# mit-han-lab/distrifuser

Measured on NVIDIA H100. Metric: SDXL 50-step latency (ms/image), lower is better.
Workload: dtype f16

## Files before the change

### distrifuser_b200/compat/unet_2d_condition.py

```python
from __future__ import annotations

import math
from types import SimpleNamespace

import torch
from torch import nn
from torch.nn import functional as F

SDXL = dict(
    in_channels=4, out_channels=4, block_out_channels=(320, 640, 1280), layers_per_block=2,
    down_block_types=("DownBlock2D", "CrossAttnDownBlock2D", "CrossAttnDownBlock2D"),
    up_block_types=("CrossAttnUpBlock2D", "CrossAttnUpBlock2D", "UpBlock2D"),
    transformer_layers_per_block=(1, 2, 10), attention_head_dim=(5, 10, 20), cross_attention_dim=2048,
    use_linear_projection=True, norm_num_groups=32, norm_eps=1e-5, addition_embed_type="text_time",
    addition_time_embed_dim=256, projection_class_embeddings_input_dim=2816, sample_size=128,
)
SD15 = dict(
    in_channels=4, out_channels=4, block_out_channels=(320, 640, 1280, 1280), layers_per_block=2,
    down_block_types=("CrossAttnDownBlock2D",) * 3 + ("DownBlock2D",),
    up_block_types=("UpBlock2D",) + ("CrossAttnUpBlock2D",) * 3,
    transformer_layers_per_block=(1, 1, 1, 1), attention_head_dim=(8, 8, 8, 8), cross_attention_dim=768,
    use_linear_projection=False, norm_num_groups=32, norm_eps=1e-5, addition_embed_type=None,
    addition_time_embed_dim=None, projection_class_embeddings_input_dim=None, sample_size=64,
)


class UNet2DConditionOutput:
    def __init__(self, sample):
        self.sample = sample

    def __getitem__(self, i):
        return (self.sample,)[i]


class Attention(nn.Module):

    def __init__(self, query_dim, cross_attention_dim, heads, dim_head):
        super().__init__()
        inner = heads * dim_head
        self.heads, self.inner_dim = heads, inner
        self.residual_connection, self.rescale_output_factor = False, 1.0
        kv_dim = query_dim if cross_attention_dim is None else cross_attention_dim
        self.to_q = nn.Linear(query_dim, inner, bias=False)
        self.to_k = nn.Linear(kv_dim, inner, bias=False)
        self.to_v = nn.Linear(kv_dim, inner, bias=False)
        self.to_out = nn.ModuleList([nn.Linear(inner, query_dim), nn.Dropout(0.0)])

    def forward(self, hidden_states, encoder_hidden_states=None, **kw):
        raise RuntimeError("Attention must be wrapped by DistriSelfAttentionPP / DistriCrossAttentionPP "
                           "(distrifuser_b200 has no unfused attention path)")


class GEGLU(nn.Module):
    def __init__(self, dim_in, dim_out):
        super().__init__()
        self.proj = nn.Linear(dim_in, dim_out * 2)
        self._fused = None
        self.norm_fused = None

    def _fused_weights(self, block):
        from .. import ops
        w, b = self.proj.weight, self.proj.bias
        key = (block, w._version, w.data_ptr(), w.dtype, w.device, None if b is None else (b._version, b.data_ptr()))
        if self._fused is None or self._fused[0] != key:
            if torch.cuda.is_current_stream_capturing():
                raise RuntimeError("GEGLU: weights changed since the last eager call; run one eager UNet call before capturing graphs")
            with torch.no_grad():
                wi, bi = ops.geglu_interleave(w.detach(), None if b is None else b.detach(), block)
            self._fused = (key, wi, bi)
        return self._fused[1], self._fused[2]

    def forward(self, x):
        if x.is_cuda and x.dtype == torch.float16:
            from .. import ops
            D, K = self.proj.out_features // 2, self.proj.in_features
            block = ops.geglu_block(x.numel() // K, 2 * D, K) if ops.use_fused_linear("geglu") else 0
            if block:
                wi, bi = self._fused_weights(block)
                return ops.linear_geglu(x, wi, bi, block)
            return ops.geglu(self.proj(x))
        y = self.proj(x)
        x, gate = y.chunk(2, dim=-1)
        return x * F.gelu(gate)


class FeedForward(nn.Module):
    def __init__(self, dim):
        super().__init__()
        self.net = nn.ModuleList([GEGLU(dim, 4 * dim), nn.Dropout(0.0), nn.Linear(4 * dim, dim)])

    def forward(self, x):
        return self.net[2](self.net[0](x))


class BasicTransformerBlock(nn.Module):
    def __init__(self, dim, heads, head_dim, cross_dim):
        super().__init__()
        self.norm1 = nn.LayerNorm(dim)
        self.attn1 = Attention(dim, None, heads, head_dim)
        self.norm2 = nn.LayerNorm(dim)
        self.attn2 = Attention(dim, cross_dim, heads, head_dim)
        self.norm3 = nn.LayerNorm(dim)
        self.ff = FeedForward(dim)

    def forward_chained(self, x, pending, encoder_hidden_states=None):
        from ..ops import add_layernorm
        x, h = add_layernorm(x, pending, self.norm1)
        x, h = add_layernorm(x, self.attn1(h, encoder_hidden_states=None), self.norm2)
        x, h = add_layernorm(x, self.attn2(h, encoder_hidden_states=encoder_hidden_states), self.norm3)
        return x, self.ff(h)

    def forward(self, x, encoder_hidden_states=None):
        if x.is_cuda and x.dtype == torch.float16:
            x, pending = self.forward_chained(x, None, encoder_hidden_states)
            return x + pending
        x = x + self.attn1(self.norm1(x), encoder_hidden_states=None)
        x = x + self.attn2(self.norm2(x), encoder_hidden_states=encoder_hidden_states)
        return x + self.ff(self.norm3(x))


class Transformer2DModel(nn.Module):
    def __init__(self, heads, head_dim, channels, depth, cross_dim, groups, linear_proj):
        super().__init__()
        inner = heads * head_dim
        self.use_linear_projection = linear_proj
        self.norm = nn.GroupNorm(groups, channels, eps=1e-6)
        self.proj_in = nn.Linear(channels, inner) if linear_proj else nn.Conv2d(channels, inner, 1)
        self.transformer_blocks = nn.ModuleList([BasicTransformerBlock(inner, heads, head_dim, cross_dim) for _ in range(depth)])
        self.proj_out = nn.Linear(inner, channels) if linear_proj else nn.Conv2d(inner, channels, 1)

    @staticmethod
    def _tokens(x):
        b, c, h, w = x.shape
        return x.permute(0, 2, 3, 1).reshape(b, h * w, c)

    @staticmethod
    def _image(t, h, w):
        b, _, c = t.shape
        return t.reshape(b, h, w, c).permute(0, 3, 1, 2)

    def forward(self, x, encoder_hidden_states=None):
        _, _, h, w = x.shape
        res = x
        x = self.norm(x)
        if self.use_linear_projection:
            t = self.proj_in(self._tokens(x))
        else:
            t = self._tokens(self.proj_in(x))
        if t.is_cuda and t.dtype == torch.float16:
            pending = None
            for blk in self.transformer_blocks:
                t, pending = blk.forward_chained(t, pending, encoder_hidden_states)
            t = t + pending
        else:
            for blk in self.transformer_blocks:
                t = blk(t, encoder_hidden_states=encoder_hidden_states)
        if self.use_linear_projection:
            x = self._image(self.proj_out(t), h, w)
        else:
            x = self.proj_out(self._image(t, h, w))
        return x + res


class ResnetBlock2D(nn.Module):
    def __init__(self, cin, cout, temb, groups, eps):
        super().__init__()
        self.norm1 = nn.GroupNorm(groups, cin, eps=eps)
        self.conv1 = nn.Conv2d(cin, cout, 3, padding=1)
        self.time_emb_proj = nn.Linear(temb, cout)
        self.norm2 = nn.GroupNorm(groups, cout, eps=eps)
        self.dropout = nn.Dropout(0.0)
        self.conv2 = nn.Conv2d(cout, cout, 3, padding=1)
        self.nonlinearity = nn.SiLU()
        self.conv_shortcut = nn.Conv2d(cin, cout, 1) if cin != cout else None
        self.output_scale_factor = 1.0
        self.fused_norm_act = False
        self.temb_proj = None
        self.temb_has_conv1_bias = False

    def folds_conv1_bias(self) -> bool:
        return self.fused_norm_act and _conv_of(self.conv1).bias is not None

    def _tail_bias(self):
        c2 = _conv_of(self.conv2)
        if self.conv_shortcut is None or self.conv_shortcut.bias is None:
            return c2.bias
        key = (c2.bias._version, self.conv_shortcut.bias._version, c2.bias.data_ptr())
        cache = getattr(self, "_tail_bias_cache", None)
        if cache is None or cache[0] != key:
            if torch.cuda.is_current_stream_capturing():
                raise RuntimeError("conv biases changed since the last eager call; run one eager UNet call before capture")
            with torch.no_grad():
                self._tail_bias_cache = cache = (key, (c2.bias.detach() + self.conv_shortcut.bias.detach()).contiguous())
        return cache[1]

    def forward(self, x, temb):
        fused_halo = self.fused_norm_act and hasattr(self.conv1, "halo_plan")
        fold1 = self.temb_proj is not None and self.temb_has_conv1_bias
        fused_tail = self.fused_norm_act and hasattr(self.conv2, "halo_plan") and x.is_cuda and x.dtype == torch.float16
        k1 = dict(fold_bias=True) if fold1 else {}
        if fused_halo and self.conv1.halo_plan(x) is not None:
            h = self.conv1.forward_padded(self.norm1(x, pad_for=self.conv1), **k1)
        else:
            h = self.norm1(x)
            if not self.fused_norm_act:
                h = self.nonlinearity(h)
            h = self.conv1(h, **k1)
        t = self.temb_proj if self.temb_proj is not None else self.time_emb_proj(self.nonlinearity(temb))
        if fused_tail:
            sc = self.conv_shortcut
            res = x if sc is None else F.conv2d(x, sc.weight)
            tail_bias = self._tail_bias()
            if fused_halo and self.conv2.halo_plan(h) is not None:
                return self.conv2.forward_padded(self.norm2(h, addend=t, pad_for=self.conv2), residual=res, bias=tail_bias)
            return self.conv2(self.norm2(h, addend=t), residual=res, bias=tail_bias)
        if fused_halo and self.conv2.halo_plan(h) is not None:
            h = self.conv2.forward_padded(self.norm2(h, addend=t, pad_for=self.conv2))
        else:
            if self.fused_norm_act:
                h = self.norm2(h, addend=t)
            else:
                h = self.nonlinearity(self.norm2(h + t[:, :, None, None]))
            h = self.conv2(h)
        if self.conv_shortcut is not None:
            x = self.conv_shortcut(x)
        return x + h


def _conv_of(m):
    return m.module if hasattr(m, "module") and isinstance(getattr(m, "module"), nn.Conv2d) else m


class Downsample2D(nn.Module):
    def __init__(self, c):
        super().__init__()
        self.conv = nn.Conv2d(c, c, 3, stride=2, padding=1)

    def forward(self, x):
        return self.conv(x)


class Upsample2D(nn.Module):
    def __init__(self, c):
        super().__init__()
        self.conv = nn.Conv2d(c, c, 3, padding=1)

    def forward(self, x):
        return self.conv(F.interpolate(x, scale_factor=2.0, mode="nearest"))


class _Down(nn.Module):
    def __init__(self, cin, cout, temb, layers, groups, eps, downsample, attn):
        super().__init__()
        self.resnets = nn.ModuleList([ResnetBlock2D(cin if i == 0 else cout, cout, temb, groups, eps) for i in range(layers)])
        if attn is not None:
            self.attentions = nn.ModuleList([Transformer2DModel(channels=cout, groups=groups, **attn) for _ in range(layers)])
        self.has_cross_attention = attn is not None
        self.downsamplers = nn.ModuleList([Downsample2D(cout)]) if downsample else None

    def forward(self, x, temb, ehs):
        skips = []
        for i, res in enumerate(self.resnets):
            x = res(x, temb)
            if self.has_cross_attention:
                x = self.attentions[i](x, encoder_hidden_states=ehs)
            skips.append(x)
        if self.downsamplers is not None:
            x = self.downsamplers[0](x)
            skips.append(x)
        return x, skips


class _Mid(nn.Module):
    def __init__(self, c, temb, groups, eps, attn):
        super().__init__()
        self.resnets = nn.ModuleList([ResnetBlock2D(c, c, temb, groups, eps) for _ in range(2)])
        self.attentions = nn.ModuleList([Transformer2DModel(channels=c, groups=groups, **attn)])

    def forward(self, x, temb, ehs):
        x = self.resnets[0](x, temb)
        x = self.attentions[0](x, encoder_hidden_states=ehs)
        return self.resnets[1](x, temb)


class _Up(nn.Module):
    def __init__(self, cin, cout, prev, temb, layers, groups, eps, upsample, attn):
        super().__init__()
        self.resnets = nn.ModuleList()
        for i in range(layers):
            skip = cin if i == layers - 1 else cout
            self.resnets.append(ResnetBlock2D((prev if i == 0 else cout) + skip, cout, temb, groups, eps))
        if attn is not None:
            self.attentions = nn.ModuleList([Transformer2DModel(channels=cout, groups=groups, **attn) for _ in range(layers)])
        self.has_cross_attention = attn is not None
        self.upsamplers = nn.ModuleList([Upsample2D(cout)]) if upsample else None

    def forward(self, x, skips, temb, ehs):
        for i, res in enumerate(self.resnets):
            x = res(torch.cat([x, skips.pop()], dim=1), temb)
            if self.has_cross_attention:
                x = self.attentions[i](x, encoder_hidden_states=ehs)
        if self.upsamplers is not None:
            x = self.upsamplers[0](x)
        return x


class TimestepEmbedding(nn.Module):
    def __init__(self, cin, dim):
        super().__init__()
        self.linear_1 = nn.Linear(cin, dim)
        self.act = nn.SiLU()
# ... 130 lines not shown
```

### distrifuser_b200/csrc/linear.cu

```cuda
#include <math.h>
#include <string.h>

#include "tc_ptx.cuh"

using namespace df;
using namespace df::tc;

namespace {

constexpr int BM = 128;
constexpr int BK = 64;
constexpr int NTHREADS = 288;
constexpr int NCONSUMER_WARPS = 8;
constexpr uint32_t A_BYTES = BM * BK * 2;

template <int BN> struct Stages { static constexpr int value = BN == 256 ? 4 : 5; };

template <int BN>
struct __align__(1024) SmemT {
  __half a[Stages<BN>::value][BM * BK];
  __half b[Stages<BN>::value][BN * BK];
  uint64_t full[Stages<BN>::value], empty[Stages<BN>::value];
};

enum { EPI_PLAIN = 0, EPI_GEGLU = 1 };

struct LinearArgs {
  const __half* bias;
  const __half* residual;
  __half* out;
  int64_t M;
  int N, K;
  int64_t ldr, ldo;
  int tiles_m, tiles_n;
  int publish;
  int pub_col0, pub_cols;
  int idx;
  uint32_t peer_mask;
  uint64_t tensor_off, slot_bytes;
  df_comm_t comm;
};

__device__ __forceinline__ float gelu_erf(float x) {
  const float z = fabsf(x) * 0.70710678118654752f;
  const float t = __fdividef(1.f, fmaf(0.3275911f, z, 1.f));
  float p = fmaf(1.061405429f, t, -1.453152027f);
  p = fmaf(p, t, 1.421413741f);
  p = fmaf(p, t, -0.284496736f);
  p = fmaf(p, t, 0.254829592f);
  const float e = p * t * __expf(-z * z);
  const float phi = x >= 0.f ? 1.f - 0.5f * e : 0.5f * e;
  return x * phi;
}

__device__ __forceinline__ float2 ld_h2f(const __half* p) { return __half22float2(*reinterpret_cast<const __half2*>(p)); }

template <int BN>
__device__ __forceinline__ void wgmma_tile(float* acc, uint64_t a_desc, uint64_t b_desc, uint32_t accumulate) {
  if constexpr (BN == 256) wgmma_ss_n256(acc, a_desc, b_desc, accumulate);
  else wgmma_ss_n160(acc, a_desc, b_desc, accumulate);
}

template <int BN>
__device__ __forceinline__ void load_tile(SmemT<BN>& sm, const void* tm_a, const void* tm_w, int tm, int tn, int kblocks,
                                          uint32_t& stage, uint32_t& phase) {
  constexpr int STAGES = Stages<BN>::value;
  constexpr uint32_t B_BYTES = BN * BK * 2;
  for (int kb = 0; kb < kblocks; ++kb) {
    mbar_wait(&sm.empty[stage], phase ^ 1u);
    mbar_expect_tx(&sm.full[stage], A_BYTES + B_BYTES);
    tma_load_2d(sm.a[stage], tm_a, &sm.full[stage], kb * BK, tm * BM);
    tma_load_2d(sm.b[stage], tm_w, &sm.full[stage], kb * BK, tn * BN);
    if (++stage == STAGES) { stage = 0; phase ^= 1u; }
  }
}

template <int BN>
__device__ __forceinline__ void mma_tile(SmemT<BN>& sm, float* acc, int wg, int lane, int kblocks, uint32_t& stage,
                                         uint32_t& phase) {
  constexpr int STAGES = Stages<BN>::value;
  fence_regs<BN / 2>(acc);
  uint32_t prev = 0;
  for (int kb = 0; kb < kblocks; ++kb) {
    mbar_wait(&sm.full[stage], phase);
    const uint32_t a_addr = smem_u32(sm.a[stage]) + wg * 64 * 128, b_addr = smem_u32(sm.b[stage]);
    wgmma_fence();
#pragma unroll
    for (int kk = 0; kk < BK / 16; ++kk)
      wgmma_tile<BN>(acc, smem_desc(a_addr + kk * 32, 16, 1024), smem_desc(b_addr + kk * 32, 16, 1024), (kb | kk) > 0);
    wgmma_commit();
    wgmma_wait<1>();
    if (kb > 0 && lane == 0) mbar_arrive(&sm.empty[prev]);
    prev = stage;
    if (++stage == STAGES) { stage = 0; phase ^= 1u; }
  }
  wgmma_wait<0>();
  fence_regs<BN / 2>(acc);
  if (lane == 0) mbar_arrive(&sm.empty[prev]);
}

template <int EPI, int BN>
__global__ void __launch_bounds__(NTHREADS, 1)
linear_kernel(const __grid_constant__ CUtensorMap tm_a, const __grid_constant__ CUtensorMap tm_w, LinearArgs p) {
  static_assert(BN % 32 == 0 && BN <= 256 && (BN * BK * 2) % 1024 == 0, "tile shape");
  constexpr int STAGES = Stages<BN>::value;
  using Smem = SmemT<BN>;
  extern __shared__ __align__(1024) uint8_t smem_raw[];
  Smem& sm = *reinterpret_cast<Smem*>(smem_raw);
  if ((smem_u32(smem_raw) & 1023u) != 0) __trap();
  const int warp = threadIdx.x >> 5, lane = threadIdx.x & 31;
  const int ntiles = p.tiles_m * p.tiles_n;
  const int kblocks = p.K / BK;

  if (threadIdx.x == 0) {
    for (int s = 0; s < STAGES; ++s) { mbar_init(&sm.full[s], 1); mbar_init(&sm.empty[s], NCONSUMER_WARPS); }
    asm volatile("fence.mbarrier_init.release.cluster;" ::: "memory");
  }
  __syncthreads();

  if (warp == NCONSUMER_WARPS) {
    if (lane == 0) {
      prefetch_tmap(&tm_a);
      prefetch_tmap(&tm_w);
      uint32_t stage = 0, phase = 0;
      for (int tile = blockIdx.x; tile < ntiles; tile += gridDim.x)
        load_tile<BN>(sm, &tm_a, &tm_w, tile % p.tiles_m, tile / p.tiles_m, kblocks, stage, phase);
    }
  } else {
    const int wg = warp >> 2;
    const int c4 = lane & 3;
    const int rloc = wg * 64 + (warp & 3) * 16 + (lane >> 2);
    uint32_t pub_epoch = 0;
    if (p.publish) pub_epoch = p.comm.clock[0];
    uint32_t stage = 0, phase = 0;
    float acc[BN / 2];
    for (int tile = blockIdx.x; tile < ntiles; tile += gridDim.x) {
      const int tm = tile % p.tiles_m, tn = tile / p.tiles_m;
      mma_tile<BN>(sm, acc, wg, lane, kblocks, stage, phase);
#pragma unroll
      for (int h = 0; h < 2; ++h) {
        const int64_t grow = (int64_t)tm * BM + rloc + 8 * h;
        if (grow >= p.M) continue;
        if (EPI == EPI_GEGLU) {
          __half* dst = p.out + grow * p.ldo + tn * (BN / 2);
#pragma unroll
          for (int i = 0; i < BN / 16; ++i) {
            const int c = 8 * i + 2 * c4;
            float2 bh = make_float2(0.f, 0.f), bg = make_float2(0.f, 0.f);
            if (p.bias) { bh = ld_h2f(p.bias + tn * BN + c); bg = ld_h2f(p.bias + tn * BN + BN / 2 + c); }
            const float* hv = acc + 4 * i + 2 * h;
            const float* gv = acc + 4 * (i + BN / 16) + 2 * h;
            const float2 hf = __half22float2(__floats2half2_rn(hv[0] + bh.x, hv[1] + bh.y));
            const float2 gf = __half22float2(__floats2half2_rn(gv[0] + bg.x, gv[1] + bg.y));
            *reinterpret_cast<__half2*>(dst + c) = __floats2half2_rn(hf.x * gelu_erf(gf.x), hf.y * gelu_erf(gf.y));
          }
        } else {
          const int col0 = tn * BN;
          __half* dst = p.out + grow * p.ldo + col0;
          const __half* res = p.residual ? p.residual + grow * p.ldr + col0 : nullptr;
#pragma unroll
          for (int i = 0; i < BN / 8; ++i) {
            const int c = 8 * i + 2 * c4;
            const int col = col0 + c;
            if (col >= p.N) continue;
            float2 f = make_float2(acc[4 * i + 2 * h], acc[4 * i + 2 * h + 1]);
            if (p.bias) { const float2 bb = ld_h2f(p.bias + col); f.x += bb.x; f.y += bb.y; }
            __half2 o = __floats2half2_rn(f.x, f.y);
            if (res) o = __hadd2(o, *reinterpret_cast<const __half2*>(res + c));
            *reinterpret_cast<__half2*>(dst + c) = o;
            if (p.publish && col >= p.pub_col0) {
              const uint64_t off = slot_offset(p.comm, pub_epoch, p.tensor_off, p.slot_bytes, p.comm.rank) +
                                   ((uint64_t)grow * p.pub_cols + (col - p.pub_col0)) * 2;
              for (int q = 0; q < p.comm.world; ++q)
                if (p.peer_mask >> q & 1) *reinterpret_cast<__half2*>((char*)p.comm.base[q] + off) = o;
            }
          }
        }
      }
    }
  }
  if (p.publish) signal_when_last(p.comm, &p.comm.tickets[p.idx], gridDim.x, p.idx, p.peer_mask, p.comm.clock[0]);
}

int make_map2d(CUtensorMap* m, const void* base, int64_t rows, int K, int64_t pitch, int box_rows) {
  EncodeTiledFn enc = tensor_map_encoder();
  DF_REQUIRE(enc != nullptr, "cuTensorMapEncodeTiled is not available from this driver");
  cuuint64_t dims[2] = {(cuuint64_t)K, (cuuint64_t)rows};
  cuuint64_t strides[1] = {(cuuint64_t)pitch * 2};
  cuuint32_t box[2] = {BK, (cuuint32_t)box_rows};
  cuuint32_t estr[2] = {1, 1};
  CUresult r = enc(m, CU_TENSOR_MAP_DATA_TYPE_FLOAT16, 2, const_cast<void*>(base), dims, strides, box, estr,
                   CU_TENSOR_MAP_INTERLEAVE_NONE, CU_TENSOR_MAP_SWIZZLE_128B, CU_TENSOR_MAP_L2_PROMOTION_L2_256B,
                   CU_TENSOR_MAP_FLOAT_OOB_FILL_NONE);
  DF_REQUIRE(r == CUDA_SUCCESS, "cuTensorMapEncodeTiled failed (%d): base=%p rows=%lld K=%d pitch=%lld", (int)r, base,
             (long long)rows, K, (long long)pitch);
  return 0;
}

template <int EPI, int BN>
int launch_linear(const CUtensorMap& ta, const CUtensorMap& tw, const LinearArgs& args, int ctas, cudaStream_t st) {
  static bool attr_set = false;
  if (!attr_set) {
    DF_CHECK_CUDA(cudaFuncSetAttribute(linear_kernel<EPI, BN>, cudaFuncAttributeMaxDynamicSharedMemorySize, (int)sizeof(SmemT<BN>)));
    attr_set = true;
  }
  linear_kernel<EPI, BN><<<ctas, NTHREADS, sizeof(SmemT<BN>), st>>>(ta, tw, args);
  DF_CHECK_LAUNCH();
  return 0;
}

double tile_cost(int64_t M, int N, int bn, int ctas_avail) {
  const long long tm = (M + BM - 1) / BM, tn = (N + bn - 1) / bn, tiles = tm * tn;
  const long long rounds = (tiles + ctas_avail - 1) / ctas_avail;
  return (double)rounds * (bn + 64);
}

}

namespace {
int pick_bn(int64_t M, int N, int epilogue, int cap) {
  const bool ok160 = epilogue == EPI_PLAIN || N % 160 == 0, ok256 = epilogue == EPI_PLAIN || N % 256 == 0;
  if (!ok256) return ok160 ? 160 : 0;
  if (ok160 && tile_cost(M, N, 160, cap) < 0.97 * tile_cost(M, N, 256, cap)) return 160;
  return 256;
}
}

extern "C" int df_linear_supported(int64_t M, int N, int K, int epilogue) {
  if (M < 1 || N < 8 || N % 8 != 0 || K < BK || K % BK != 0) return 0;
  if (epilogue == EPI_GEGLU && pick_bn(M, N, epilogue, sm_count()) == 0) return 0;
  return 1;
}

extern "C" int df_linear_geglu_block(int64_t M, int N, int K) {
  (void)K;
  const int bn = pick_bn(M, N, EPI_GEGLU, sm_count());
  return bn / 2;
}

extern "C" int df_linear_fwd(df_comm_t comm, const void* a, const void* w, const void* bias, const void* residual, void* out,
                             int64_t M, int N, int K, int64_t lda, int64_t ldw, int64_t ldr, int64_t ldo, int epilogue,
                             int geglu_block, int publish, int pub_col0, int idx, uint32_t peer_mask, uint64_t tensor_off,
                             uint64_t slot_bytes, int max_ctas, void* stream) {
  DF_REQUIRE(epilogue == EPI_PLAIN || epilogue == EPI_GEGLU, "df_linear_fwd: unknown epilogue %d", epilogue);
  DF_REQUIRE(df_linear_supported(M, N, K, epilogue), "df_linear_fwd: unsupported shape M=%lld N=%d K=%d (N %% 8, K %% 64%s)",
             (long long)M, N, K, epilogue == EPI_GEGLU ? ", GEGLU: N % 256" : "");
  DF_REQUIRE(((uintptr_t)a % 16) == 0 && ((uintptr_t)w % 16) == 0 && ((uintptr_t)out % 16) == 0 && ((uintptr_t)bias % 16) == 0 &&
                 ((uintptr_t)residual % 16) == 0 && lda % 8 == 0 && ldw % 8 == 0 && ldo % 8 == 0 && ldr % 8 == 0,
             "df_linear_fwd: operands must be 16-byte aligned with pitches multiple of 8");
  DF_REQUIRE(!(publish && epilogue != EPI_PLAIN), "df_linear_fwd: publication is a plain-epilogue feature");
  LinearArgs args;
  memset(&args, 0, sizeof(args));
  args.bias = (const __half*)bias; args.residual = (const __half*)residual; args.out = (__half*)out;
  args.M = M; args.N = N; args.K = K; args.ldr = ldr; args.ldo = ldo;
  const int sms = sm_count();
  const int cap = max_ctas > 0 ? max_ctas : sms;
  int bn = pick_bn(M, N, epilogue, epilogue == EPI_GEGLU ? sms : cap);
  if (epilogue == EPI_GEGLU && geglu_block > 0) {
    DF_REQUIRE(geglu_block == 80 || geglu_block == 128, "df_linear_fwd: geglu_block must be 80 or 128");
    bn = 2 * geglu_block;
    DF_REQUIRE(N % bn == 0, "df_linear_fwd: interleave block %d does not tile N=%d", geglu_block, N);
  }
  args.tiles_m = (int)((M + BM - 1) / BM);
  args.tiles_n = (N + bn - 1) / bn;
  args.publish = publish && peer_mask != 0;
  args.comm = comm;
  if (args.publish) {
    DF_REQUIRE(pub_col0 >= 0 && pub_col0 < N && pub_col0 % 8 == 0, "df_linear_fwd: bad pub_col0");
    args.pub_col0 = pub_col0; args.pub_cols = N - pub_col0; args.idx = idx; args.peer_mask = peer_mask;
    args.tensor_off = tensor_off; args.slot_bytes = slot_bytes;
    DF_REQUIRE((uint64_t)M * args.pub_cols * 2 <= slot_bytes, "df_linear_fwd: published columns larger than the slot");
  }
  int ctas = args.tiles_m * args.tiles_n;
  if (ctas > cap) ctas = cap;
  if (ctas < 1) ctas = 1;
  CUtensorMap ta, tw;
  if (int rc = make_map2d(&ta, a, M, K, lda, BM)) return rc;
  if (int rc = make_map2d(&tw, w, N, K, ldw, bn)) return rc;
  cudaStream_t st = (cudaStream_t)stream;
  if (epilogue == EPI_GEGLU) {
    if (bn == 160) return launch_linear<EPI_GEGLU, 160>(ta, tw, args, ctas, st);
    return launch_linear<EPI_GEGLU, 256>(ta, tw, args, ctas, st);
  }
  if (bn == 160) return launch_linear<EPI_PLAIN, 160>(ta, tw, args, ctas, st);
  return launch_linear<EPI_PLAIN, 256>(ta, tw, args, ctas, st);
}

namespace {
constexpr int ZC_BN = 160;

struct ZeroConvProblem {
  const __half* bias;
  __half* out;
  int M, N, tiles_m, tile0, kblocks;
};

struct ZeroConvArgs {
  CUtensorMap a[DF_ZERO_CONV_MAX_PROBLEMS], w[DF_ZERO_CONV_MAX_PROBLEMS];
  ZeroConvProblem p[DF_ZERO_CONV_MAX_PROBLEMS];
  const float* scale;
  int nproblems, ntiles;
};
static_assert(sizeof(ZeroConvArgs) <= 4096, "the problem list must fit the 4 KiB kernel parameter space");

__device__ __forceinline__ int zc_problem(const ZeroConvArgs& z, int tile) {
  int q = 0;
  while (q + 1 < z.nproblems && tile >= z.p[q + 1].tile0) ++q;
  return q;
}

__global__ void __launch_bounds__(NTHREADS, 1) zero_conv_kernel(const __grid_constant__ ZeroConvArgs z) {
  constexpr int BN = ZC_BN;
  constexpr int STAGES = Stages<BN>::value;
  using Smem = SmemT<BN>;
  extern __shared__ __align__(1024) uint8_t smem_raw[];
  Smem& sm = *reinterpret_cast<Smem*>(smem_raw);
  if ((smem_u32(smem_raw) & 1023u) != 0) __trap();
  const int warp = threadIdx.x >> 5, lane = threadIdx.x & 31;

  if (threadIdx.x == 0) {
    for (int s = 0; s < STAGES; ++s) { mbar_init(&sm.full[s], 1); mbar_init(&sm.empty[s], NCONSUMER_WARPS); }
    asm volatile("fence.mbarrier_init.release.cluster;" ::: "memory");
  }
  __syncthreads();

  if (warp == NCONSUMER_WARPS) {
    if (lane == 0) {
      uint32_t stage = 0, phase = 0;
      for (int tile = blockIdx.x; tile < z.ntiles; tile += gridDim.x) {
        const int q = zc_problem(z, tile);
        const ZeroConvProblem& p = z.p[q];
        const int t = tile - p.tile0;
        load_tile<BN>(sm, &z.a[q], &z.w[q], t % p.tiles_m, t / p.tiles_m, p.kblocks, stage, phase);
      }
    }
  } else {
    const int wg = warp >> 2;
    const int c4 = lane & 3;
    const int rloc = wg * 64 + (warp & 3) * 16 + (lane >> 2);
    const float scale = *z.scale;
    uint32_t stage = 0, phase = 0;
    float acc[BN / 2];
    for (int tile = blockIdx.x; tile < z.ntiles; tile += gridDim.x) {
      const ZeroConvProblem& p = z.p[zc_problem(z, tile)];
      const int t = tile - p.tile0;
      const int tm = t % p.tiles_m, tn = t / p.tiles_m;
      mma_tile<BN>(sm, acc, wg, lane, p.kblocks, stage, phase);
#pragma unroll
      for (int h = 0; h < 2; ++h) {
        const int64_t grow = (int64_t)tm * BM + rloc + 8 * h;
        if (grow >= p.M) continue;
        const int col0 = tn * BN;
        __half* dst = p.out + grow * p.N + col0;
#pragma unroll
        for (int i = 0; i < BN / 8; ++i) {
          const int c = 8 * i + 2 * c4;
          const int col = col0 + c;
          if (col >= p.N) continue;
          float2 f = make_float2(acc[4 * i + 2 * h], acc[4 * i + 2 * h + 1]);
          if (p.bias) { const float2 bb = ld_h2f(p.bias + col); f.x += bb.x; f.y += bb.y; }
          const float2 r = __half22float2(__floats2half2_rn(f.x, f.y));
          *reinterpret_cast<__half2*>(dst + c) = __floats2half2_rn(r.x * scale, r.y * scale);
        }
      }
    }
  }
}
}

extern "C" int df_controlnet_zero_convs(int nproblems, const void* const* x_host, const void* const* w_host,
                                        const void* const* bias_host, void* const* out_host, const int64_t* m_host,
                                        const int32_t* n_host, const int32_t* k_host, const float* scale, int max_ctas,
                                        void* stream) {
  DF_REQUIRE(nproblems >= 1 && nproblems <= DF_ZERO_CONV_MAX_PROBLEMS, "df_controlnet_zero_convs: %d problems (1..%d)",
             nproblems, DF_ZERO_CONV_MAX_PROBLEMS);
  DF_REQUIRE(x_host && w_host && out_host && m_host && n_host && k_host && scale, "df_controlnet_zero_convs: null argument");
  DF_REQUIRE(((uintptr_t)scale % 4) == 0, "df_controlnet_zero_convs: scale must be a 4-byte aligned fp32");
  ZeroConvArgs z;
  memset(&z, 0, sizeof(z));
  int ntiles = 0;
  for (int i = 0; i < nproblems; ++i) {
    const int64_t M = m_host[i];
    const int N = n_host[i], K = k_host[i];
    const void* bias = bias_host ? bias_host[i] : nullptr;
    DF_REQUIRE(M >= 1 && M <= INT32_MAX && N >= 8 && N % 8 == 0 && K >= 8 && K % 8 == 0,
               "df_controlnet_zero_convs: problem %d has unsupported shape M=%lld N=%d K=%d (N %% 8, K %% 8)", i,
               (long long)M, N, K);
    DF_REQUIRE(x_host[i] && w_host[i] && out_host[i] && ((uintptr_t)x_host[i] % 16) == 0 &&
                   ((uintptr_t)w_host[i] % 16) == 0 && ((uintptr_t)out_host[i] % 16) == 0 && ((uintptr_t)bias % 16) == 0,
               "df_controlnet_zero_convs: problem %d: operands must be non-null and 16-byte aligned", i);
    if (int rc = make_map2d(&z.a[i], x_host[i], M, K, K, BM)) return rc;
    if (int rc = make_map2d(&z.w[i], w_host[i], N, K, K, ZC_BN)) return rc;
    ZeroConvProblem& p = z.p[i];
    p.bias = (const __half*)bias; p.out = (__half*)out_host[i];
    p.M = (int)M; p.N = N; p.kblocks = (K + BK - 1) / BK;
    p.tiles_m = (int)((M + BM - 1) / BM);
    p.tile0 = ntiles;
    const int64_t t = (int64_t)p.tiles_m * ((N + ZC_BN - 1) / ZC_BN);
    DF_REQUIRE(ntiles + t <= INT32_MAX, "df_controlnet_zero_convs: too many tiles");
    ntiles += (int)t;
  }
  z.scale = scale; z.nproblems = nproblems; z.ntiles = ntiles;
  const int cap = max_ctas > 0 ? max_ctas : sm_count();
  const int ctas = ntiles < cap ? ntiles : cap;
  static bool attr_set = false;
  if (!attr_set) {
    DF_CHECK_CUDA(cudaFuncSetAttribute(zero_conv_kernel, cudaFuncAttributeMaxDynamicSharedMemorySize, (int)sizeof(SmemT<ZC_BN>)));
    attr_set = true;
  }
  zero_conv_kernel<<<ctas, NTHREADS, sizeof(SmemT<ZC_BN>), (cudaStream_t)stream>>>(z);
  DF_CHECK_LAUNCH();
  return 0;
}
```

### distrifuser_b200/modules/pp/attn.py

```python
import ctypes as C

import torch
from torch import nn
from torch.nn import functional as F

from ... import _lib
from ...utils import DistriConfig
from ..base_module import BaseModule, nvtx_range


_WORKSPACES: dict = {}


def _shared_workspace(device, nbytes: int) -> torch.Tensor:
    lst = _WORKSPACES.setdefault(device, [])
    if not lst or lst[-1].numel() < nbytes:
        if torch.cuda.is_current_stream_capturing():
            raise RuntimeError("attention workspace would grow during CUDA-graph capture; run one eager UNet call first")
        lst.append(torch.zeros(max(nbytes, 16 << 20), dtype=torch.uint8, device=device))
    return lst[-1]


class DistriAttentionPP(BaseModule):
    def __init__(self, module: nn.Module, distri_config: DistriConfig):
        super().__init__(module, distri_config)
        to_k, to_v = module.to_k, module.to_v
        assert isinstance(to_k, nn.Linear) and isinstance(to_v, nn.Linear)
        assert (to_k.bias is None) == (to_v.bias is None)
        assert to_k.weight.shape == to_v.weight.shape
        in_size, out_size = to_k.in_features, to_k.out_features
        to_kv = nn.Linear(in_size, out_size * 2, bias=to_k.bias is not None, device=to_k.weight.device,
                          dtype=to_k.weight.dtype)
        with torch.no_grad():
            to_kv.weight[:out_size].copy_(to_k.weight)
            to_kv.weight[out_size:].copy_(to_v.weight)
            if to_k.bias is not None:
                to_kv.bias[:out_size].copy_(to_k.bias)
                to_kv.bias[out_size:].copy_(to_v.bias)
        self.to_kv = to_kv
        self._kvmaps = None

    def _attend(self, q, kv_own, lens, own_seg, wait_flags, kind="self", scale=0.0, real_width=None):
        attn = self.module
        b, lq, Cq = q.shape
        heads = attn.heads
        d = Cq // heads
        out = torch.empty((b, lq, Cq), dtype=q.dtype, device=q.device)
        cm = self.comm_manager
        nseg = len(lens)
        if nseg > 1:
            comm, maps = cm.group, self._kvmaps.data_ptr()
        else:
            comm, maps = _lib.null_comm(), None
        seg_rank = (C.c_int32 * _lib.MAX_WORLD)(*range(_lib.MAX_WORLD))
        seg_len = _lib.int32_array(lens)
        L = _lib.lib()
        ws_bytes = L.df_attn_workspace_bytes_ragged(b, lq, seg_len, nseg, heads, d)
        ws = _shared_workspace(q.device, ws_bytes).data_ptr() if ws_bytes else None
        prof = _lib.PROFILE
        if prof is not None:
            e0, e1 = torch.cuda.Event(enable_timing=True), torch.cuda.Event(enable_timing=True)
            e0.record()
        _lib.check(L.df_attn_fwd_ragged(comm, q.data_ptr(), kv_own.data_ptr(), out.data_ptr(), maps, b, lq, seg_len,
                                        heads, d, q.stride(1), kv_own.stride(1), out.stride(1), nseg, own_seg,
                                        seg_rank, self.idx or 0, int(wait_flags), float(scale), ws, ws_bytes,
                                        torch.cuda.current_stream().cuda_stream), "df_attn_fwd_ragged")
        if prof is not None:
            e1.record()
            prof.append(dict(kernel="fmha_fwd_kernel", kind=kind,
                             flops=4.0 * b * lq * sum(lens) * (real_width or Cq),
                             bytes=2.0 * (2 * b * lq * Cq + b * sum(lens) * 2 * Cq),
                             shape=(b, lq, sum(lens), heads, d), start=e0, end=e1))
        return out

    def _project_out(self, hidden_states, residual, weight=None):
        attn = self.module
        if weight is not None:
            hidden_states = F.linear(hidden_states, weight, attn.to_out[0].bias)
        else:
            hidden_states = attn.to_out[0](hidden_states)
        hidden_states = attn.to_out[1](hidden_states)
        if attn.residual_connection:
            hidden_states = hidden_states + residual
        if attn.rescale_output_factor != 1.0:
            hidden_states = hidden_states / attn.rescale_output_factor
        return hidden_states


class DistriCrossAttentionPP(DistriAttentionPP):
    def __init__(self, module: nn.Module, distri_config: DistriConfig):
        super().__init__(module, distri_config)
        self.kv_cache = None

    @nvtx_range("DistriCrossAttentionPP")
    def forward(self, hidden_states, encoder_hidden_states=None, scale: float = 1.0, *args, **kwargs):
        assert encoder_hidden_states is not None
        self._require_cuda_half(hidden_states, "DistriCrossAttentionPP")
        attn = self.module
        q = attn.to_q(hidden_states)
        if self.counter == 0 or self.kv_cache is None:
            kv = self.to_kv(encoder_hidden_states)
            if self.kv_cache is not None and self.kv_cache.shape == kv.shape:
                self.kv_cache.copy_(kv)
            else:
                self.kv_cache = kv
        kv = self.kv_cache
        out = self._attend(q, kv, [kv.shape[1]], 0, False, kind="cross")
        out = self._project_out(out, hidden_states)
        self.counter += 1
        return out


class DistriSelfAttentionPP(DistriAttentionPP):
    def __init__(self, module: nn.Module, distri_config: DistriConfig):
        super().__init__(module, distri_config)
        self._w_qkv = None
        self._w_qkv_key = None
        self._w_out = None
        self._head_pad = 0

    def _qkv_weight(self, dtype):
        to_q, to_kv = self.module.to_q, self.to_kv
        if not (isinstance(to_q, nn.Linear) and to_q.bias is None and to_kv.bias is None and
                to_q.in_features == to_kv.in_features and to_q.out_features * 2 == to_kv.out_features and
                to_q.weight.dtype == dtype and to_kv.weight.dtype == dtype):
            return None
        wq, wkv, wo = to_q.weight, to_kv.weight, self.module.to_out[0].weight
        heads = self.module.heads
        d = to_q.out_features // heads
        pad = 64 if d < 64 else 0
        key = (wq._version, wkv._version, wo._version, wq.data_ptr(), wkv.data_ptr(), wo.data_ptr(), wq.device, dtype, pad)
        if key != self._w_qkv_key:
            if torch.cuda.is_current_stream_capturing():
                raise RuntimeError("DistriSelfAttentionPP: attention weights changed since the last eager call; run one "
                                   "eager UNet call (pipeline.prepare()) before capturing CUDA graphs")
            with torch.no_grad():
                if pad:
                    cin = wq.shape[1]
                    widen = lambda w: F.pad(w.detach().reshape(-1, heads, d, cin), (0, 0, 0, pad - d)).reshape(-1, cin)
                    self._w_qkv = torch.cat([widen(wq), widen(wkv)], 0).contiguous()
                    self._w_out = F.pad(wo.detach().reshape(wo.shape[0], heads, d), (0, pad - d)).reshape(wo.shape[0], heads * pad).contiguous()
                else:
                    self._w_qkv = torch.cat([wq.detach(), wkv.detach()], 0).contiguous()
                    self._w_out = None
            self._w_qkv_key = key
            self._head_pad = pad
        return self._w_qkv

    @nvtx_range("DistriSelfAttentionPP")
    def forward(self, hidden_states, encoder_hidden_states=None, scale: float = 1.0, *args, **kwargs):
        cfg = self.distri_config
        self._require_cuda_half(hidden_states, "DistriSelfAttentionPP")
        attn = self.module
        n, r = cfg.n_device_per_batch, cfg.split_idx()
        b, l, c = hidden_states.shape
        cm = self.comm_manager
        w_qkv = self._qkv_weight(hidden_states.dtype)
        heads = attn.heads
        d_real = c // heads
        padded = w_qkv is not None and self._head_pad != 0
        cs = heads * self._head_pad if padded else c
        lens = self.patch_rows(l) if n > 1 else [l]
        if n > 1 and self._recording() and self.idx is None:
            self.idx = cm.register_tensor((b, l, 2 * cs), hidden_states.dtype, layer_type="attn",
                                          slot_bytes=b * max(lens) * 2 * cs * hidden_states.element_size())
        live = n > 1 and self._bound()
        sync = live and (cfg.mode == "full_sync" or self._is_sync_step())
        ship = live and (sync or cfg.mode != "no_sync")
        published = False
        if w_qkv is not None:
            from ... import ops
            if not padded and ops.use_fused_linear("qkv") and ops.linear_supported(b * l, 3 * c, c):
                pub = (cm.group, c, self.idx, cm.peers_mask(), cm.tensor_off[self.idx], cm.slot_bytes[self.idx]) if ship else None
                qkv = ops.linear(hidden_states, w_qkv, publish=pub)
                published = ship
            else:
                qkv = F.linear(hidden_states, w_qkv)
            q, kv = qkv[..., :cs], qkv[..., cs:]
        else:
            q = attn.to_q(hidden_states)
            kv = self.to_kv(hidden_states)
        sm_scale = d_real ** -0.5 if padded else 0.0
        if not live:
            out = self._attend(q, kv, [l], 0, False, scale=sm_scale, real_width=c)
        else:
            if self._kvmaps is None:
                self._kvmaps = torch.empty(_lib.NBANKS * n * _lib.TENSORMAP_BYTES, dtype=torch.uint8, device=q.device)
                _lib.check(_lib.lib().df_attn_make_kvmaps_ragged(cm.group, cm.tensor_off[self.idx], cm.slot_bytes[self.idx], b,
                                                                 _lib.int32_array(lens), heads, cs // heads,
                                                                 self._kvmaps.data_ptr(), torch.cuda.current_stream().cuda_stream),
                           "df_attn_make_kvmaps_ragged")
            if ship and not published:
                cm.enqueue(self.idx, kv, async_stream=not sync)
            out = self._attend(q, kv, lens, r, True, scale=sm_scale, real_width=c)
        out = self._project_out(out, hidden_states, self._w_out if padded else None)
        self.counter += 1
        return out
```

### distrifuser_b200/ops.py

```python
import os as _os

import torch

from . import _lib


def geglu(y: torch.Tensor) -> torch.Tensor:
    assert y.is_cuda and y.dtype == torch.float16 and y.stride(-1) == 1
    cols = y.shape[-1] // 2
    y2 = y.reshape(-1, 2 * cols)
    out = torch.empty((*y.shape[:-1], cols), dtype=y.dtype, device=y.device)
    _lib.check(_lib.lib().df_geglu(y2.data_ptr(), out.data_ptr(), y2.shape[0], cols, y2.stride(0), cols,
                                   torch.cuda.current_stream().cuda_stream), "df_geglu")
    return out


def add_layernorm(x: torch.Tensor, r: torch.Tensor | None, norm: torch.nn.LayerNorm):
    assert x.is_cuda and x.dtype == torch.float16
    C = x.shape[-1]
    x = x.contiguous()
    y = torch.empty_like(x)
    if r is not None:
        r = r.contiguous()
        s = torch.empty_like(x)
    else:
        s = x
    _lib.check(_lib.lib().df_add_layernorm(x.data_ptr(), r.data_ptr() if r is not None else None,
                                           s.data_ptr() if r is not None else None, y.data_ptr(), norm.weight.data_ptr(),
                                           norm.bias.data_ptr(), x.numel() // C, C, float(norm.eps),
                                           torch.cuda.current_stream().cuda_stream), "df_add_layernorm")
    return s, y


def conv2d_bias_residual(x: torch.Tensor, conv: torch.nn.Conv2d, padding, residual: torch.Tensor | None = None,
                         bias: torch.Tensor | None = None, fold_bias: bool = False) -> torch.Tensor:
    import torch.nn.functional as F
    b = conv.bias if bias is None else bias
    ok = (x.is_cuda and x.dtype == torch.float16 and conv.out_channels % 8 == 0 and
          x.is_contiguous(memory_format=torch.channels_last))
    if not ok:
        out = F.conv2d(x, conv.weight, None if fold_bias else b, stride=conv.stride, padding=padding)
        return out if residual is None else residual + out
    out = F.conv2d(x, conv.weight, None, stride=conv.stride, padding=padding)
    if (b is None or fold_bias) and residual is None:
        return out
    if not out.is_contiguous(memory_format=torch.channels_last):
        out = out.contiguous(memory_format=torch.channels_last)
    if b is None or fold_bias:
        return residual + out
    if residual is not None:
        assert residual.shape == out.shape and residual.dtype == out.dtype
        if not residual.is_contiguous(memory_format=torch.channels_last):
            residual = residual.contiguous(memory_format=torch.channels_last)
    n, c, h, w = out.shape
    _lib.check(_lib.lib().df_bias_residual_add(out.data_ptr(), residual.data_ptr() if residual is not None else None,
                                               b.data_ptr(), out.data_ptr(), n * h * w, c,
                                               torch.cuda.current_stream().cuda_stream), "df_bias_residual_add")
    return out



_FUSED_LINEAR = set(_os.environ.get("DF_LINEAR", "geglu").replace("all", "geglu,qkv,out,ff2,proj").split(","))


def use_fused_linear(kind: str) -> bool:
    return kind in _FUSED_LINEAR


GEGLU_BLOCK = 128


def linear_supported(M: int, N: int, K: int, geglu: bool = False) -> bool:
    return bool(_lib.lib().df_linear_supported(M, N, K, 1 if geglu else 0))


def geglu_block(M: int, two_d: int, K: int) -> int:
    if not linear_supported(M, two_d, K, geglu=True):
        return 0
    return int(_lib.lib().df_linear_geglu_block(M, two_d, K))


def geglu_interleave(weight: torch.Tensor, bias: torch.Tensor | None, block: int = GEGLU_BLOCK):
    two_d, K = weight.shape
    D = two_d // 2
    assert D % block == 0
    w = torch.stack([weight[:D].reshape(D // block, block, K), weight[D:].reshape(D // block, block, K)], 1)
    w = w.reshape(two_d, K).contiguous()
    b = None
    if bias is not None:
        b = torch.stack([bias[:D].reshape(-1, block), bias[D:].reshape(-1, block)], 1).reshape(two_d).contiguous()
    return w, b


def linear(x: torch.Tensor, weight: torch.Tensor, bias: torch.Tensor | None = None, residual: torch.Tensor | None = None,
           out: torch.Tensor | None = None, publish=None) -> torch.Tensor:
    assert x.is_cuda and x.dtype == torch.float16 and weight.dtype == torch.float16 and x.stride(-1) == 1 and weight.stride(-1) == 1
    K = x.shape[-1]
    N = weight.shape[0]
    x2 = x.reshape(-1, K)
    M = x2.shape[0]
    if out is None:
        out = torch.empty((*x.shape[:-1], N), dtype=x.dtype, device=x.device)
    o2 = out.view(-1, N)
    r2 = residual.reshape(-1, N) if residual is not None else None
    if publish is not None:
        comm, pub_col0, idx, mask, off, sb = publish
    else:
        comm, pub_col0, idx, mask, off, sb = _lib.null_comm(), 0, 0, 0, 0, 0
    _lib.check(_lib.lib().df_linear_fwd(comm, x2.data_ptr(), weight.data_ptr(), bias.data_ptr() if bias is not None else None,
                                        r2.data_ptr() if r2 is not None else None, o2.data_ptr(), M, N, K, x2.stride(0),
                                        weight.stride(0), r2.stride(0) if r2 is not None else 0, o2.stride(0), 0, 0,
                                        int(publish is not None), pub_col0, idx, mask, off, sb, 0,
                                        torch.cuda.current_stream().cuda_stream), "df_linear_fwd")
    return out


def linear_geglu(x: torch.Tensor, w_interleaved: torch.Tensor, b_interleaved: torch.Tensor | None, block: int = GEGLU_BLOCK) -> torch.Tensor:
    assert x.is_cuda and x.dtype == torch.float16 and x.stride(-1) == 1
    K = x.shape[-1]
    N = w_interleaved.shape[0]
    x2 = x.reshape(-1, K)
    out = torch.empty((*x.shape[:-1], N // 2), dtype=x.dtype, device=x.device)
    _lib.check(_lib.lib().df_linear_fwd(_lib.null_comm(), x2.data_ptr(), w_interleaved.data_ptr(),
                                        b_interleaved.data_ptr() if b_interleaved is not None else None, None, out.data_ptr(),
                                        x2.shape[0], N, K, x2.stride(0), w_interleaved.stride(0), 0, N // 2, 1, block, 0, 0, 0, 0, 0, 0, 0,
                                        torch.cuda.current_stream().cuda_stream), "df_linear_fwd")
    return out


def controlnet_zero_convs(xs, convs, scale: torch.Tensor) -> list[torch.Tensor]:
    import ctypes as C
    n = len(xs)
    assert len(convs) == n and scale.is_cuda and scale.dtype == torch.float32 and scale.numel() == 1
    outs, xp, wp, bp, op, ms, ns, ks = [], [], [], [], [], [], [], []
    for x, conv in zip(xs, convs):
        assert x.is_cuda and x.dtype == torch.float16 and tuple(conv.kernel_size) == (1, 1)
        x = x.contiguous(memory_format=torch.channels_last)
        b, k, h, w = x.shape
        out = torch.empty((b, conv.out_channels, h, w), dtype=x.dtype, device=x.device, memory_format=torch.channels_last)
        outs.append(out)
        xp.append(x.data_ptr()); wp.append(conv.weight.data_ptr()); op.append(out.data_ptr())
        bp.append(conv.bias.data_ptr() if conv.bias is not None else None)
        ms.append(b * h * w); ns.append(conv.out_channels); ks.append(k)
    ptrs = lambda v: (C.c_void_p * n)(*v)
    _lib.check(_lib.lib().df_controlnet_zero_convs(n, ptrs(xp), ptrs(wp), ptrs(bp), ptrs(op), (C.c_int64 * n)(*ms),
                                                   (C.c_int32 * n)(*ns), (C.c_int32 * n)(*ks), scale.data_ptr(), 0,
                                                   torch.cuda.current_stream().cuda_stream), "df_controlnet_zero_convs")
    return outs
```

Before: 1596.

## Add warp-specialized staged epilogue to linear kernel and route projections through it

```diff
diff --git a/distrifuser_b200/compat/unet_2d_condition.py b/distrifuser_b200/compat/unet_2d_condition.py
--- a/distrifuser_b200/compat/unet_2d_condition.py
+++ b/distrifuser_b200/compat/unet_2d_condition.py
@@ -90,7 +90,8 @@
         self.net = nn.ModuleList([GEGLU(dim, 4 * dim), nn.Dropout(0.0), nn.Linear(4 * dim, dim)])
 
     def forward(self, x):
-        return self.net[2](self.net[0](x))
+        from .. import ops
+        return ops.project("ff2", self.net[0](x), self.net[2])
 
 
 class BasicTransformerBlock(nn.Module):
@@ -144,7 +145,8 @@
         res = x
         x = self.norm(x)
         if self.use_linear_projection:
-            t = self.proj_in(self._tokens(x))
+            from .. import ops
+            t = ops.project("proj", self._tokens(x), self.proj_in)
         else:
             t = self._tokens(self.proj_in(x))
         if t.is_cuda and t.dtype == torch.float16:
@@ -156,7 +158,7 @@
             for blk in self.transformer_blocks:
                 t = blk(t, encoder_hidden_states=encoder_hidden_states)
         if self.use_linear_projection:
-            x = self._image(self.proj_out(t), h, w)
+            x = self._image(ops.project("proj", t, self.proj_out), h, w)
         else:
             x = self.proj_out(self._image(t, h, w))
         return x + res
diff --git a/distrifuser_b200/csrc/linear.cu b/distrifuser_b200/csrc/linear.cu
--- a/distrifuser_b200/csrc/linear.cu
+++ b/distrifuser_b200/csrc/linear.cu
@@ -10,17 +10,30 @@
 
 constexpr int BM = 128;
 constexpr int BK = 64;
-constexpr int NTHREADS = 288;
 constexpr int NCONSUMER_WARPS = 8;
+constexpr int NCONSUMERS = 32 * NCONSUMER_WARPS;
+constexpr int NTHREADS = NCONSUMERS + 128;
+constexpr int NEPILOGUE = 96;
+constexpr int NTHREADS_ZC = NCONSUMERS + 32;
+constexpr int CONSUMER_REGS = 208, WG2_REGS = 88;
 constexpr uint32_t A_BYTES = BM * BK * 2;
 
-template <int BN> struct Stages { static constexpr int value = BN == 256 ? 4 : 5; };
+template <int BN> struct Stages { static constexpr int value = BN == 256 ? 3 : 5; };
 
 template <int BN>
 struct __align__(1024) SmemT {
   __half a[Stages<BN>::value][BM * BK];
   __half b[Stages<BN>::value][BN * BK];
   uint64_t full[Stages<BN>::value], empty[Stages<BN>::value];
+};
+
+template <int BN> __host__ __device__ constexpr int stage_pitch() { return BN + 8; }
+
+template <int BN>
+struct __align__(1024) LinearSmem {
+  SmemT<BN> ring;
+  __half stg[BM * stage_pitch<BN>()];
+  uint64_t stg_full, stg_empty;
 };
 
 enum { EPI_PLAIN = 0, EPI_GEGLU = 1 };
@@ -55,6 +68,16 @@
 
 __device__ __forceinline__ float2 ld_h2f(const __half* p) { return __half22float2(*reinterpret_cast<const __half2*>(p)); }
 
+__device__ __forceinline__ void stmatrix_x4(uint32_t addr, uint32_t r0, uint32_t r1, uint32_t r2, uint32_t r3) {
+  asm volatile("stmatrix.sync.aligned.m8n8.x4.shared.b16 [%0], {%1, %2, %3, %4};" ::"r"(addr), "r"(r0), "r"(r1), "r"(r2), "r"(r3)
+               : "memory");
+}
+
+union H8 {
+  uint4 u;
+  __half2 h[4];
+};
+
 template <int BN>
 __device__ __forceinline__ void wgmma_tile(float* acc, uint64_t a_desc, uint64_t b_desc, uint32_t accumulate) {
   if constexpr (BN == 256) wgmma_ss_n256(acc, a_desc, b_desc, accumulate);
@@ -104,7 +127,8 @@
 linear_kernel(const __grid_constant__ CUtensorMap tm_a, const __grid_constant__ CUtensorMap tm_w, LinearArgs p) {
   static_assert(BN % 32 == 0 && BN <= 256 && (BN * BK * 2) % 1024 == 0, "tile shape");
   constexpr int STAGES = Stages<BN>::value;
-  using Smem = SmemT<BN>;
+  constexpr int SP = stage_pitch<BN>();
+  using Smem = LinearSmem<BN>;
   extern __shared__ __align__(1024) uint8_t smem_raw[];
   Smem& sm = *reinterpret_cast<Smem*>(smem_raw);
   if ((smem_u32(smem_raw) & 1023u) != 0) __trap();
@@ -113,69 +137,107 @@
   const int kblocks = p.K / BK;
 
   if (threadIdx.x == 0) {
-    for (int s = 0; s < STAGES; ++s) { mbar_init(&sm.full[s], 1); mbar_init(&sm.empty[s], NCONSUMER_WARPS); }
+    for (int s = 0; s < STAGES; ++s) { mbar_init(&sm.ring.full[s], 1); mbar_init(&sm.ring.empty[s], NCONSUMER_WARPS); }
+    mbar_init(&sm.stg_full, NCONSUMERS);
+    mbar_init(&sm.stg_empty, NEPILOGUE);
     asm volatile("fence.mbarrier_init.release.cluster;" ::: "memory");
   }
   __syncthreads();
 
-  if (warp == NCONSUMER_WARPS) {
-    if (lane == 0) {
-      prefetch_tmap(&tm_a);
-      prefetch_tmap(&tm_w);
-      uint32_t stage = 0, phase = 0;
-      for (int tile = blockIdx.x; tile < ntiles; tile += gridDim.x)
-        load_tile<BN>(sm, &tm_a, &tm_w, tile % p.tiles_m, tile / p.tiles_m, kblocks, stage, phase);
+  if (warp < NCONSUMER_WARPS) {
+    setmaxnreg_inc<CONSUMER_REGS>();
+    const int wg = warp >> 2;
+    const int c4 = lane & 3;
+    const int mrow = wg * 64 + (warp & 3) * 16 + ((lane >> 3) & 1) * 8 + (lane & 7);
+    const uint32_t st_addr = smem_u32(sm.stg) + (uint32_t)(mrow * SP + (lane >> 4) * 8) * 2u;
+    uint32_t stage = 0, phase = 0, sphase = 0;
+    float acc[BN / 2];
+    for (int tile = blockIdx.x; tile < ntiles; tile += gridDim.x) {
+      const int tn = tile / p.tiles_m;
+      __half2 bias2[BN / 8];
+#pragma unroll
+      for (int i = 0; i < BN / 8; ++i) {
+        const int col = tn * BN + 8 * i + 2 * c4;
+        bias2[i] = p.bias && col < p.N ? *reinterpret_cast<const __half2*>(p.bias + col) : __float2half2_rn(0.f);
+      }
+      mma_tile<BN>(sm.ring, acc, wg, lane, kblocks, stage, phase);
+      mbar_wait(&sm.stg_empty, sphase ^ 1u);
+#pragma unroll
+      for (int j = 0; j < BN / 16; ++j) {
+        uint32_t r[4];
+#pragma unroll
+        for (int q = 0; q < 2; ++q) {
+          const int i = 2 * j + q;
+          const float2 bb = __half22float2(bias2[i]);
+          r[2 * q] = pack_h2(acc[4 * i] + bb.x, acc[4 * i + 1] + bb.y);
+          r[2 * q + 1] = pack_h2(acc[4 * i + 2] + bb.x, acc[4 * i + 3] + bb.y);
+        }
+        stmatrix_x4(st_addr + j * 32, r[0], r[1], r[2], r[3]);
+      }
+      mbar_arrive(&sm.stg_full);
+      sphase ^= 1u;
     }
   } else {
-    const int wg = warp >> 2;
-    const int c4 = lane & 3;
-    const int rloc = wg * 64 + (warp & 3) * 16 + (lane >> 2);
-    uint32_t pub_epoch = 0;
-    if (p.publish) pub_epoch = p.comm.clock[0];
-    uint32_t stage = 0, phase = 0;
-    float acc[BN / 2];
-    for (int tile = blockIdx.x; tile < ntiles; tile += gridDim.x) {
-      const int tm = tile % p.tiles_m, tn = tile / p.tiles_m;
-      mma_tile<BN>(sm, acc, wg, lane, kblocks, stage, phase);
-#pragma unroll
-      for (int h = 0; h < 2; ++h) {
-        const int64_t grow = (int64_t)tm * BM + rloc + 8 * h;
-        if (grow >= p.M) continue;
+    setmaxnreg_dec<WG2_REGS>();
+    if (warp == NCONSUMER_WARPS) {
+      if (lane == 0) {
+        prefetch_tmap(&tm_a);
+        prefetch_tmap(&tm_w);
+        uint32_t stage = 0, phase = 0;
+        for (int tile = blockIdx.x; tile < ntiles; tile += gridDim.x)
+          load_tile<BN>(sm.ring, &tm_a, &tm_w, tile % p.tiles_m, tile / p.tiles_m, kblocks, stage, phase);
+      }
+    } else {
+      const int et = threadIdx.x - (NCONSUMERS + 32);
+      uint32_t pub_epoch = 0;
+      if (p.publish) pub_epoch = p.comm.clock[0];
+      uint32_t sphase = 0;
+      for (int tile = blockIdx.x; tile < ntiles; tile += gridDim.x) {
+        const int tm = tile % p.tiles_m, tn = tile / p.tiles_m;
+        mbar_wait(&sm.stg_full, sphase);
         if (EPI == EPI_GEGLU) {
-          __half* dst = p.out + grow * p.ldo + tn * (BN / 2);
-#pragma unroll
-          for (int i = 0; i < BN / 16; ++i) {
-            const int c = 8 * i + 2 * c4;
-            float2 bh = make_float2(0.f, 0.f), bg = make_float2(0.f, 0.f);
-            if (p.bias) { bh = ld_h2f(p.bias + tn * BN + c); bg = ld_h2f(p.bias + tn * BN + BN / 2 + c); }
-            const float* hv = acc + 4 * i + 2 * h;
-            const float* gv = acc + 4 * (i + BN / 16) + 2 * h;
-            const float2 hf = __half22float2(__floats2half2_rn(hv[0] + bh.x, hv[1] + bh.y));
-            const float2 gf = __half22float2(__floats2half2_rn(gv[0] + bg.x, gv[1] + bg.y));
-            *reinterpret_cast<__half2*>(dst + c) = __floats2half2_rn(hf.x * gelu_erf(gf.x), hf.y * gelu_erf(gf.y));
+          constexpr int CH = BN / 16;
+          for (int v = et; v < BM * CH; v += NEPILOGUE) {
+            const int r = v / CH, c = v % CH;
+            const int64_t grow = (int64_t)tm * BM + r;
+            if (grow >= p.M) continue;
+            H8 hv, gv, o;
+            hv.u = *reinterpret_cast<const uint4*>(sm.stg + r * SP + 8 * c);
+            gv.u = *reinterpret_cast<const uint4*>(sm.stg + r * SP + 8 * (c + CH));
+#pragma unroll
+            for (int k = 0; k < 4; ++k) {
+              const float2 hf = __half22float2(hv.h[k]), gf = __half22float2(gv.h[k]);
+              o.h[k] = __floats2half2_rn(hf.x * gelu_erf(gf.x), hf.y * gelu_erf(gf.y));
+            }
+            *reinterpret_cast<uint4*>(p.out + grow * p.ldo + tn * (BN / 2) + 8 * c) = o.u;
           }
         } else {
-          const int col0 = tn * BN;
-          __half* dst = p.out + grow * p.ldo + col0;
-          const __half* res = p.residual ? p.residual + grow * p.ldr + col0 : nullptr;
-#pragma unroll
-          for (int i = 0; i < BN / 8; ++i) {
-            const int c = 8 * i + 2 * c4;
-            const int col = col0 + c;
-            if (col >= p.N) continue;
-            float2 f = make_float2(acc[4 * i + 2 * h], acc[4 * i + 2 * h + 1]);
-            if (p.bias) { const float2 bb = ld_h2f(p.bias + col); f.x += bb.x; f.y += bb.y; }
-            __half2 o = __floats2half2_rn(f.x, f.y);
-            if (res) o = __hadd2(o, *reinterpret_cast<const __half2*>(res + c));
-            *reinterpret_cast<__half2*>(dst + c) = o;
+          constexpr int CH = BN / 8;
+#pragma unroll 4
+          for (int v = et; v < BM * CH; v += NEPILOGUE) {
+            const int r = v / CH, c = v % CH;
+            const int64_t grow = (int64_t)tm * BM + r;
+            const int col = tn * BN + 8 * c;
+            if (grow >= p.M || col >= p.N) continue;
+            H8 o;
+            o.u = *reinterpret_cast<const uint4*>(sm.stg + r * SP + 8 * c);
+            if (p.residual) {
+              H8 rv;
+              rv.u = __ldg(reinterpret_cast<const uint4*>(p.residual + grow * p.ldr + col));
+#pragma unroll
+              for (int k = 0; k < 4; ++k) o.h[k] = __hadd2(o.h[k], rv.h[k]);
+            }
+            *reinterpret_cast<uint4*>(p.out + grow * p.ldo + col) = o.u;
             if (p.publish && col >= p.pub_col0) {
               const uint64_t off = slot_offset(p.comm, pub_epoch, p.tensor_off, p.slot_bytes, p.comm.rank) +
                                    ((uint64_t)grow * p.pub_cols + (col - p.pub_col0)) * 2;
               for (int q = 0; q < p.comm.world; ++q)
-                if (p.peer_mask >> q & 1) *reinterpret_cast<__half2*>((char*)p.comm.base[q] + off) = o;
+                if (p.peer_mask >> q & 1) *reinterpret_cast<uint4*>((char*)p.comm.base[q] + off) = o.u;
             }
           }
         }
+        mbar_arrive(&sm.stg_empty);
+        sphase ^= 1u;
       }
     }
   }
@@ -201,10 +263,10 @@
 int launch_linear(const CUtensorMap& ta, const CUtensorMap& tw, const LinearArgs& args, int ctas, cudaStream_t st) {
   static bool attr_set = false;
   if (!attr_set) {
-    DF_CHECK_CUDA(cudaFuncSetAttribute(linear_kernel<EPI, BN>, cudaFuncAttributeMaxDynamicSharedMemorySize, (int)sizeof(SmemT<BN>)));
+    DF_CHECK_CUDA(cudaFuncSetAttribute(linear_kernel<EPI, BN>, cudaFuncAttributeMaxDynamicSharedMemorySize, (int)sizeof(LinearSmem<BN>)));
     attr_set = true;
   }
-  linear_kernel<EPI, BN><<<ctas, NTHREADS, sizeof(SmemT<BN>), st>>>(ta, tw, args);
+  linear_kernel<EPI, BN><<<ctas, NTHREADS, sizeof(LinearSmem<BN>), st>>>(ta, tw, args);
   DF_CHECK_LAUNCH();
   return 0;
 }
@@ -267,6 +329,7 @@
   args.comm = comm;
   if (args.publish) {
     DF_REQUIRE(pub_col0 >= 0 && pub_col0 < N && pub_col0 % 8 == 0, "df_linear_fwd: bad pub_col0");
+    DF_REQUIRE(tensor_off % 16 == 0 && slot_bytes % 16 == 0, "df_linear_fwd: slots must be 16-byte aligned");
     args.pub_col0 = pub_col0; args.pub_cols = N - pub_col0; args.idx = idx; args.peer_mask = peer_mask;
     args.tensor_off = tensor_off; args.slot_bytes = slot_bytes;
     DF_REQUIRE((uint64_t)M * args.pub_cols * 2 <= slot_bytes, "df_linear_fwd: published columns larger than the slot");
@@ -309,7 +372,7 @@
   return q;
 }
 
-__global__ void __launch_bounds__(NTHREADS, 1) zero_conv_kernel(const __grid_constant__ ZeroConvArgs z) {
+__global__ void __launch_bounds__(NTHREADS_ZC, 1) zero_conv_kernel(const __grid_constant__ ZeroConvArgs z) {
   constexpr int BN = ZC_BN;
   constexpr int STAGES = Stages<BN>::value;
   using Smem = SmemT<BN>;
@@ -408,7 +471,7 @@
     DF_CHECK_CUDA(cudaFuncSetAttribute(zero_conv_kernel, cudaFuncAttributeMaxDynamicSharedMemorySize, (int)sizeof(SmemT<ZC_BN>)));
     attr_set = true;
   }
-  zero_conv_kernel<<<ctas, NTHREADS, sizeof(SmemT<ZC_BN>), (cudaStream_t)stream>>>(z);
+  zero_conv_kernel<<<ctas, NTHREADS_ZC, sizeof(SmemT<ZC_BN>), (cudaStream_t)stream>>>(z);
   DF_CHECK_LAUNCH();
   return 0;
 }
diff --git a/distrifuser_b200/modules/pp/attn.py b/distrifuser_b200/modules/pp/attn.py
--- a/distrifuser_b200/modules/pp/attn.py
+++ b/distrifuser_b200/modules/pp/attn.py
@@ -74,11 +74,9 @@
         return out
 
     def _project_out(self, hidden_states, residual, weight=None):
+        from ... import ops
         attn = self.module
-        if weight is not None:
-            hidden_states = F.linear(hidden_states, weight, attn.to_out[0].bias)
-        else:
-            hidden_states = attn.to_out[0](hidden_states)
+        hidden_states = ops.project("out", hidden_states, attn.to_out[0], weight)
         hidden_states = attn.to_out[1](hidden_states)
         if attn.residual_connection:
             hidden_states = hidden_states + residual
@@ -97,7 +95,8 @@
         assert encoder_hidden_states is not None
         self._require_cuda_half(hidden_states, "DistriCrossAttentionPP")
         attn = self.module
-        q = attn.to_q(hidden_states)
+        from ... import ops
+        q = ops.project("qkv", hidden_states, attn.to_q)
         if self.counter == 0 or self.kv_cache is None:
             kv = self.to_kv(encoder_hidden_states)
             if self.kv_cache is not None and self.kv_cache.shape == kv.shape:
diff --git a/distrifuser_b200/ops.py b/distrifuser_b200/ops.py
--- a/distrifuser_b200/ops.py
+++ b/distrifuser_b200/ops.py
@@ -115,6 +115,19 @@
     return out
 
 
+def project(kind: str, x: torch.Tensor, lin: torch.nn.Linear, weight: torch.Tensor | None = None) -> torch.Tensor:
+    w = lin.weight if weight is None else weight
+    K = x.shape[-1]
+    if (use_fused_linear(kind) and x.is_cuda and x.dtype == torch.float16 and w.dtype == torch.float16 and
+            x.stride(-1) == 1 and w.stride(-1) == 1 and getattr(lin, "lora_layer", None) is None and
+            linear_supported(x.numel() // K, w.shape[0], K)):
+        return linear(x, w, lin.bias)
+    if weight is None:
+        return lin(x)
+    import torch.nn.functional as F
+    return F.linear(x, weight, lin.bias)
+
+
 def linear_geglu(x: torch.Tensor, w_interleaved: torch.Tensor, b_interleaved: torch.Tensor | None, block: int = GEGLU_BLOCK) -> torch.Tensor:
     assert x.is_cuda and x.dtype == torch.float16 and x.stride(-1) == 1
     K = x.shape[-1]
```

After: 1543 (median of 6 runs). -3.3%, faster.
